# Michaelszeng/GCS-ADMM

Measured on AMD Instinct MI355X. Metric: admm_iterations_per_sec, higher is better.
Workload: dtype f64

## Files before the change

gcs_admm_amd/csrc/vertex_wg.h:

```cpp
#pragma once
#include <type_traits>

#include "gcs_math.h"
#include "step_args.h"
#include "warm_start.h"

#if defined(__HIP_DEVICE_COMPILE__)
#define WG_DEVICE 1
#else
#define WG_DEVICE 0
#endif

namespace gcs_wg {

using gcs_math::rcp;
using gcs_math::rcp1;
using gcs_math::rsqrt_nr;
using gcs_math::sqrt_nr;

#ifndef GCS_WG_THREADS
#define GCS_WG_THREADS 256
#endif
constexpr int WG_THREADS = GCS_WG_THREADS;
constexpr int WG_WAVES = WG_THREADS / 64;
// ... 160 lines not shown

struct alignas(8) WgF2 { float a, b; };

template <class T> struct WgArgs : gcsadmm_k::StepArgs<T> {
    int n_vtx;
    const int *vtx;
    const double *prox_q = nullptr, *prox_c = nullptr;
    const int *order = nullptr;
    int *unit_iters = nullptr;
};

struct Red3 { double mn, s1, s2; };

#if WG_DEVICE
template <int SH> __device__ __forceinline__ double dpp_row_shr(double x, double ident)
{
    const int ilo = __double2loint(ident), ihi = __double2hiint(ident);
    const int lo = __builtin_amdgcn_update_dpp(ilo, __double2loint(x), 0x110 + SH, 0xf, 0xf, false);
    const int hi = __builtin_amdgcn_update_dpp(ihi, __double2hiint(x), 0x110 + SH, 0xf, 0xf, false);
    return __hiloint2double(hi, lo);
}
__device__ __forceinline__ double lane_bcast(double x, int lane)
{
    return __hiloint2double(__builtin_amdgcn_readlane(__double2hiint(x), lane), __builtin_amdgcn_readlane(__double2loint(x), lane));
}
#endif

GCS_HD double wg_uniform(double x)
{
#if WG_DEVICE
    return __hiloint2double(__builtin_amdgcn_readfirstlane(__double2hiint(x)), __builtin_amdgcn_readfirstlane(__double2loint(x)));
#else
    return x;
#endif
}
GCS_HD int wg_uniform(int x)
{
#if WG_DEVICE
    return __builtin_amdgcn_readfirstlane(x);
#else
    return x;
#endif
}

template <bool VM = false> GCS_HD Red3 wg_reduce(Red3 v, double *red, int &phase)
{
#if WG_DEVICE
    v.mn = fmin(v.mn, dpp_row_shr<1>(v.mn, 1e300)); v.s1 += dpp_row_shr<1>(v.s1, 0.0); v.s2 += dpp_row_shr<1>(v.s2, 0.0);
    v.mn = fmin(v.mn, dpp_row_shr<2>(v.mn, 1e300)); v.s1 += dpp_row_shr<2>(v.s1, 0.0); v.s2 += dpp_row_shr<2>(v.s2, 0.0);
    v.mn = fmin(v.mn, dpp_row_shr<4>(v.mn, 1e300)); v.s1 += dpp_row_shr<4>(v.s1, 0.0); v.s2 += dpp_row_shr<4>(v.s2, 0.0);
    v.mn = fmin(v.mn, dpp_row_shr<8>(v.mn, 1e300)); v.s1 += dpp_row_shr<8>(v.s1, 0.0); v.s2 += dpp_row_shr<8>(v.s2, 0.0);
    Red3 w;
    w.mn = fmin(fmin(lane_bcast(v.mn, 15), lane_bcast(v.mn, 31)), fmin(lane_bcast(v.mn, 47), lane_bcast(v.mn, 63)));
    w.s1 = (lane_bcast(v.s1, 15) + lane_bcast(v.s1, 31)) + (lane_bcast(v.s1, 47) + lane_bcast(v.s1, 63));
    w.s2 = (lane_bcast(v.s2, 15) + lane_bcast(v.s2, 31)) + (lane_bcast(v.s2, 47) + lane_bcast(v.s2, 63));
    double *buf = red + phase * (3 * WG_WAVES);
    phase = phase == 2 ? 0 : phase + 1;
    const int wave = (int)threadIdx.x >> 6;
    if (((int)threadIdx.x & 63) == 0) { buf[wave * 3 + 0] = w.mn; buf[wave * 3 + 1] = w.s1; buf[wave * 3 + 2] = w.s2; }
    wg_barrier<VM>();
    Red3 r{buf[0], buf[1], buf[2]};
#pragma unroll
    for (int q = 1; q < WG_WAVES; ++q) { r.mn = fmin(r.mn, buf[3 * q]); r.s1 += buf[3 * q + 1]; r.s2 += buf[3 * q + 2]; }
    return r;
#else
    (void)red; (void)phase;
    return v;
#endif
}

GCS_HD void tri_decode(int t, int &r, int &c)
{
    r = (int)((sqrtf(8.0f * (float)t + 1.0f) - 1.0f) * 0.5f);
    if ((r + 1) * (r + 2) / 2 <= t) ++r;
    if (r * (r + 1) / 2 > t) --r;
    c = t - r * (r + 1) / 2;
}

GCS_HD int fdiv(int x, float inv) { return (int)(((float)x + 0.5f) * inv); }

GCS_HD constexpr int pki(int i, int j) { return i * (i + 1) / 2 + j; }

template <int DIM> GCS_HD void wave_ldl(double *Mq, double *rd)
{
    static_assert(DIM <= 64, "one row per lane");
#if WG_DEVICE
    const int lane = wg_tid() & 63, row = lane < DIM ? lane : DIM - 1;
    double a[DIM];
#pragma unroll
    for (int j = 0; j < DIM; ++j) a[j] = Mq[row * DIM + j];
    const double od = Mq[row * DIM + row];
    double myr = 0.0;
#pragma unroll
    for (int k = 0; k < DIM; ++k) {
        double dk = lane_bcast(a[k], k);
        const double odk = lane_bcast(od, k);
        if (!(dk > CHOL_SKIP * odk)) dk = odk > 0.0 ? CHOL_SKIP * odk : 1.0;
        const double rk = rcp(dk), col = a[k], l = col * rk;
        a[k] = l;
        if (lane == k) myr = rk;
#pragma unroll
        for (int j = k + 1; j < DIM; ++j) a[j] -= l * lane_bcast(col, j);
    }
    if (lane < DIM) {
#pragma unroll
        for (int j = 0; j < DIM - 1; ++j) Mq[lane * DIM + j] = a[j];
        rd[lane] = myr;
    }
#else
    double od[DIM], col[DIM];
    for (int k = 0; k < DIM; ++k) od[k] = Mq[k * DIM + k];
    for (int k = 0; k < DIM; ++k) {
        double dk = Mq[k * DIM + k];
        if (!(dk > CHOL_SKIP * od[k])) dk = od[k] > 0.0 ? CHOL_SKIP * od[k] : 1.0;
        const double rk = rcp(dk);
        rd[k] = rk;
        for (int i = k + 1; i < DIM; ++i) col[i] = Mq[i * DIM + k];
        for (int i = k + 1; i < DIM; ++i) {
            const double l = col[i] * rk;
            Mq[i * DIM + k] = l;
            for (int j = k + 1; j <= i; ++j) Mq[i * DIM + j] -= l * col[j];
        }
    }
#endif
}

template <int DIM> GCS_HD void wave_ldl_solve(const double *Mq, const double *rd, const double *b, double *x)
{
#if WG_DEVICE
    const int lane = wg_tid() & 63, row = lane < DIM ? lane : DIM - 1;
    double l[DIM], v = b[row];
#pragma unroll
    for (int k = 0; k < DIM - 1; ++k) l[k] = k < row ? Mq[row * DIM + k] : 0.0;
#pragma unroll
    for (int k = 0; k < DIM - 1; ++k) v -= l[k] * lane_bcast(v, k);
    v *= rd[row];
#pragma unroll
    for (int k = 1; k < DIM; ++k) l[k] = k > row ? Mq[k * DIM + row] : 0.0;
#pragma unroll
    for (int k = DIM - 1; k >= 1; --k) v -= l[k] * lane_bcast(v, k);
    if (lane < DIM) x[lane] = v;
#else
    double v[DIM];
    for (int i = 0; i < DIM; ++i) v[i] = b[i];
    for (int k = 0; k < DIM - 1; ++k)
        for (int i = k + 1; i < DIM; ++i) v[i] -= Mq[i * DIM + k] * v[k];
    for (int i = 0; i < DIM; ++i) v[i] *= rd[i];
    for (int k = DIM - 1; k >= 1; --k)
        for (int i = 0; i < k; ++i) v[i] -= Mq[k * DIM + i] * v[k];
    for (int i = 0; i < DIM; ++i) x[i] = v[i];
#endif
}

template <int DIM, bool LOWREG> GCS_HD void ldl_inverse_col(const double *Lm, const double *rd, int c, double *out, int ldo)
{
    double x[DIM];
#pragma unroll
    for (int i = 0; i < DIM; ++i) {
        double s = (i == c) ? 1.0 : 0.0;
#pragma unroll
        for (int k = 0; k < i; ++k) s -= Lm[i * DIM + k] * x[k];
        x[i] = s;
        if constexpr (DIM > 9) WG_FENCE();
    }
#pragma unroll
    for (int i = DIM - 1; i >= 0; --i) {
        double s = x[i] * rd[i];
#pragma unroll
        for (int k = i + 1; k < DIM; ++k) s -= Lm[k * DIM + i] * x[k];
        x[i] = s;
        if constexpr (LOWREG) out[i * ldo + c] = s;
        if constexpr (DIM > 9) WG_FENCE();
    }
    if constexpr (!LOWREG) {
#pragma unroll
        for (int i = 0; i < DIM; ++i) out[i * ldo + c] = x[i];
    }
}

template <int Q> GCS_HD bool soc_scaling_wb(const double *s, const double *z, double *wb, double &eta)
{
    const double ss = gcs_math::soc_det<Q>(s), zz = gcs_math::soc_det<Q>(z);
    if (!(ss > 0.0) || !(zz > 0.0)) return false;
    const double is = rsqrt_nr(ss), iz = rsqrt_nr(zz);
    double dot = 0;
    for (int k = 0; k < Q; ++k) dot += (s[k] * is) * (z[k] * iz);
    const double ig2 = 0.5 * rsqrt_nr(0.5 * (1.0 + dot));
    wb[0] = (s[0] * is + z[0] * iz) * ig2;
    for (int k = 1; k < Q; ++k) wb[k] = (s[k] * is - z[k] * iz) * ig2;
    eta = sqrt_nr((ss * is) * iz);
    return true;
}

template <int Q> GCS_HD void soc_apply_W(const double *wb, double eta, const double *x, double *y)
{
    double dd = 0;
#pragma unroll
    for (int k = 1; k < Q; ++k) dd += wb[k] * x[k];
    const double f = x[0] + dd * rcp(1.0 + wb[0]);
    y[0] = eta * (wb[0] * x[0] + dd);
#pragma unroll
    for (int k = 1; k < Q; ++k) y[k] = eta * (x[k] + wb[k] * f);
}
template <int Q> GCS_HD void soc_apply_Wi(const double *wb, double eta, const double *x, double *y)
{
    double dd = 0;
#pragma unroll
    for (int k = 1; k < Q; ++k) dd += wb[k] * x[k];
    const double ieta = rcp(eta), f = -x[0] + dd * rcp(1.0 + wb[0]);
    y[0] = ieta * (wb[0] * x[0] - dd);
#pragma unroll
    for (int k = 1; k < Q; ++k) y[k] = ieta * (x[k] + wb[k] * f);
}
template <int Q> GCS_HD void soc_apply_W2(const double *wb, double eta, const double *x, double *y)
{
    double vx = wb[0] * x[0];
#pragma unroll
    for (int k = 1; k < Q; ++k) vx -= wb[k] * x[k];
    const double ieta = rcp(eta), ie2 = ieta * ieta;
    y[0] = ie2 * (2.0 * wb[0] * vx - x[0]);
#pragma unroll
    for (int k = 1; k < Q; ++k) y[k] = ie2 * (x[k] - 2.0 * wb[k] * vx);
}

#define WG_ROWS_BEGIN_(pl, DS)                                                                                                 \
    WG_FOR_AT(rt_, (BOX ? U * 2 * N : U * m2), (pl).at(BOX ? U * 2 * N : U * m2)) {                                            \
        int u, i, jk_;                                                                                                         \
        if constexpr (BOX) { u = rt_ / (2 * N); const int ik_ = rt_ - u * (2 * N); i = ik_ / N; jk_ = ik_ - i * N; }           \
        else { u = fdiv(rt_, inv_m2); const int rem_ = rt_ - u * m2; i = rem_ >= m; jk_ = rem_ - i * m; }                      \
        double *un = UN(u);                                                                                                    \
        double ap_ = 0, ax_ = 0, adp_ = 0, adx_ = 0;                                                                           \
        if constexpr (BOX) {                                                                                                   \
            ap_ = un[W::P + i * N + jk_]; ax_ = sm[W::XV + i * N + jk_];                                                       \
            if (DS) { adp_ = un[W::DW + i * N + jk_]; adx_ = sm[W::DX + i * N + jk_]; }                                        \
        } else {                                                                                                               \
            _Pragma("unroll") for (int k_ = 0; k_ < N; ++k_) {                                                                 \
                const double a_ = A[jk_ * N + k_];                                                                             \
                ap_ += a_ * un[W::P + i * N + k_]; ax_ += a_ * sm[W::XV + i * N + k_];                                         \
                if (DS) { adp_ += a_ * un[W::DW + i * N + k_]; adx_ += a_ * sm[W::DX + i * N + k_]; }                          \
            }                                                                                                                  \
        }                                                                                                                      \
        const double yy_ = un[W::P + 2 * N], dy_ = DS ? un[W::DW + 2 * N] : 0.0;                                               \
        _Pragma("unroll") for (int rq_ = 0; rq_ < (BOX ? 4 : 2); ++rq_) {                                                      \
            const int ty = BOX ? rq_ >> 1 : rq_, j = BOX ? jk_ + (rq_ & 1) * N : jk_, ro = ty * m2 + i * m + j;                \
            const double sg_ = (BOX && (rq_ & 1)) ? -1.0 : 1.0, b_ = BC[j];                                                    \
            const double s = ty == 0 ? b_ * yy_ - sg_ * ap_ : b_ * (1.0 - yy_) - sg_ * (ax_ - ap_);                            \
            const double ds = ty == 0 ? b_ * dy_ - sg_ * adp_ : -(b_ * dy_) - sg_ * (adx_ - adp_);                             \
            (void)ds;
#define WG_ROWS_BEGIN(pl) WG_ROWS_BEGIN_(pl, false)
#define WG_ROWS_BEGIN_DS(pl) WG_ROWS_BEGIN_(pl, true)
#define WG_ROWS_END() }}

template <int N, class T, bool BOX = false, bool SPLIT = false>
GCS_HD void wg_solve_vertex(const WgArgs<T> &a, int v, double rho, double mu_scale, double *sm, int &status_out, int &iters_out,
                            double *units = nullptr)
{
    using D = WD<N>;
    using SO = WSoc<N>;
    using W = std::conditional_t<BOX, WLBox<N>, WL<N>>;
    constexpr int NW = D::NW, NX = D::NX, NB1 = D::NB1, Q = D::Q, NS = D::NS, TA = D::TA;
#ifndef GCS_WG_CONE_PAIR_MAXN
#define GCS_WG_CONE_PAIR_MAXN 3
#endif
    constexpr bool CONE_PAIR = N <= GCS_WG_CONE_PAIR_MAXN;
    const bool prox = a.prox_q != nullptr;
    const int lo = a.inc_ptr[v], d = prox ? 0 : a.inc_ptr[v + 1] - lo, d_in = prox ? 0 : a.deg_in[v], d_out = d - d_in;
    const bool sides = d > 0;
    const int p0 = a.poly_ptr[v], m = a.poly_ptr[v + 1] - p0;
    const int U = d + 1, R = 4 * m, m2 = 2 * m;
    const int US = W::unit_stride(m);
    const float inv_m2 = 1.0f / (float)m2;
    double *const UB = SPLIT ? units : sm + W::FIXED;
    auto UN = [&](int u) -> double * { return UB + u * US; };
    constexpr bool WG_VM = SPLIT;
    const int oLAM = W::ROWS, oR1 = W::ROWS + R, oR2 = W::ROWS + 2 * R;
    double *const PA = sm + W::FIXED + (SPLIT ? 0 : pad2(U * US));
    const double *A = PA, *BC = PA + pad2(m * N), *CEN = sm + W::CEN;
    double *SOC = sm + W::SOC, *SC = sm + W::SC;
    int red_phase = 0;
    WG_STAMP_INIT();
    const int deg = (4 * m + 2) * (d + 1) + 1;
    const double inv_deg = 1.0 / (double)deg;
    auto side_of = [&](int u) { return (u - 1) >= d_in ? 1 : 0; };
    auto side_lo = [&](int s) { return s ? d_in + 1 : 1; };
    auto side_hi = [&](int s) { return s ? d : d_in; };

    using WR = gcs_ws::WRec<N>;
    double *const wrec = (a.warm != nullptr && !prox) ? a.warm + a.warm_ptr[v] : nullptr;
    const int WUS = WR::unit_stride(m);
    double dtm = 0.0;
    Place pl0;
    WG_FOR_AT(t, d * NW, pl0.at(d * NW)) {
        const int e = t / NW, w = t - e * NW, edge = a.inc_edge[lo + e];
        const bool out = e >= d_in;
        const int inc = gcsadmm_k::state_column(a, lo, e, edge, out);
        double *un = UN(e + 1);
        const double Tw = gcsadmm_k::consensus_target(a, w, edge, inc, mu_scale);
        int slot = -1;
        if (w == 2 * N) slot = 2 * N;
        else if (out) slot = w;
        else if (w < N) { un[W::TF + w] = Tw; un[W::TG + N + w] = 0.0; }
        else slot = w - N;
        if (slot >= 0) {
            un[W::TG + slot] = Tw;
            if (wrec) dtm = fmax(dtm, fabs(Tw - wrec[WR::UNITS + (e + 1) * WUS + WR::TG + slot]));
        }
    }
    WG_FOR_AT(t, m * N, pl0.at(m * N)) PA[t] = a.poly_A[(size_t)p0 * N + t];
    WG_FOR_AT(j, m + N, pl0.at(m + N)) {
        if (j < m) PA[pad2(m * N) + j] = a.poly_bc[p0 + j];
        else sm[W::CEN + (j - m)] = a.center[(size_t)v * N + (j - m)];
    }
    if (prox) {
        WG_FOR(k, NX + NW) {
            sm[W::PQ + k] = a.prox_q[(size_t)v * (NX + NW) + k];
            sm[W::PC + k] = a.prox_c[(size_t)v * (NX + NW) + k];
        }
    }
    bool use_warm = false;
    double mu_ref = gcs_ws::WS_COLD_REF, ws_dT = -1.0;
    if (wrec) {
        const Red3 rt = wg_reduce<WG_VM>(Red3{-dtm, 0.0, 0.0}, sm + W::RED, red_phase);
        const bool comparable = wg_uniform((int)(wrec[0] == 1.0 && wrec[1] == rho)) != 0;
        ws_dT = wg_uniform(comparable ? -rt.mn * rho : -1.0);
        use_warm = wg_uniform((int)(comparable && ws_dT <= gcs_ws::ws_theta(wrec))) != 0;
        if (use_warm) mu_ref = wg_uniform(fmax(gcs_ws::WS_MU_MIN, gcs_ws::WS_KAPPA * ws_dT));
    }
    const bool ws_started_warm = use_warm;
    const float inv_R2 = 1.0f / (float)(R / 2);

    WG_STAMP(0);
    auto gval = [&](const double *un, int u, int k, bool wk) {
        double g = un[W::G0 + k];
        if (wk) {
            g += un[W::GU + k];
            if (u == 0 && k < 2 * N) g += k < N ? -SOC[SO::KS + 1 + k] : SOC[SO::KS + 1 + (k - N)];
        }
        return g;
    };
    auto te_tasks = [&](Place &pl, bool wk) {
        WG_FOR_AT(t, d * NW, pl.at(d * NW)) {
            const int u = 1 + t / NW, i = t - (u - 1) * NW;
            double *un = UN(u);
            double s = 0;
            if constexpr (BOX) {
                double wg = 0;
#pragma unroll
                for (int k = 0; k < NW; ++k) wg += un[W::BW + k] * gval(un, u, k, wk);
                s = -(un[W::BRS] * un[W::BW + i]) * wg;
                if (i < 2 * N) s -= un[W::BD + i] * gval(un, u, i, wk);
            } else {
#pragma unroll
                for (int k = 0; k < NW; ++k) s -= un[W::B + i * NW + k] * gval(un, u, k, wk);
            }
            un[W::TE + i] = s;
        }
    };
    auto bg_tasks = [&](Place &pl) {
        WG_FOR_AT(t, 2 * NW, pl.at(2 * NW)) {
            const int s = t / NW, i = t - s * NW;
            double acc = 0;
#pragma unroll 4
            for (int u = side_lo(s); u <= side_hi(s); ++u) acc += UN(u)[W::TE + i];
            sm[W::BG + t] = acc;
        }
        WG_FOR_AT(t, 2 * NX, pl.at(2 * NX)) {
            const int part = t / NX, c = t - part * NX, h = c / N;
            const int ulo = part ? 1 + d / 2 : 1, uhi = part ? d : d / 2;
            double acc = 0;
#pragma unroll 2
            for (int u = ulo; u <= uhi; ++u) {
                const double *un = UN(u);
                if constexpr (BOX) acc += un[W::XD + c] * un[W::TE + c] + un[W::XY + c] * un[W::TE + 2 * N];
                else {
#pragma unroll
                    for (int k = 0; k < N; ++k) acc += un[W::X + (h * N + k) * NX + c] * un[W::TE + h * N + k];
                    acc += un[W::X + 2 * N * NX + c] * un[W::TE + 2 * N];
                }
            }
            sm[W::XBG + t] = acc;
        }
    };
    auto v_tasks = [&](Place &pl) {
        WG_FOR_AT(t, 2 * NW, pl.at(2 * NW)) {
            const int s = t / NW, i = t - s * NW;
            const double *Bsi = sm + W::BSI + s * NW * NW;
            double acc = 0;
#pragma unroll
            for (int k = 0; k < NW; ++k) acc += Bsi[i * NW + k] * (sm[W::RP + s * NW + k] - sm[W::BG + s * NW + k]);
            sm[W::VV + t] = acc;
        }
    };
    auto rhs_tasks = [&](Place &pl, bool wk) {
        const double *u0 = UN(0);
        auto base_z = [&](int i) { return -gval(u0, 0, i, wk) - sm[W::VV + i] - sm[W::VV + NW + i]; };
        WG_FOR_AT(q, NX, pl.at(NX)) {
            double r = -REG_DELTA * sm[W::XV + q] - sm[W::XBG + q] - sm[W::XBG + NX + q];
            if (prox) r -= sm[W::PQ + q] * (sm[W::XV + q] + CEN[q < N ? q : q - N] - sm[W::PC + q]);
            if (wk) r -= sm[W::SOL + q];
            for (int s = 0; s < 2; ++s) {
                const double *BXs = sm + W::BXS + s * NW * NX;
#pragma unroll
                for (int i = 0; i < NW; ++i) r -= BXs[i * NX + q] * sm[W::VV + s * NW + i];
            }
            sm[W::RHS + q] = r;
        }
        WG_FOR_AT(k, N, pl.at(N))
            sm[W::RHS + NX + k] = base_z(k) + SOC[SO::CV + k] * SC[SC_GT] * rcp(SC[SC_C0]);
        WG_FOR_AT(k, N, pl.at(N))
            sm[W::RHS + NX + N + k] = base_z(k) + base_z(N + k);
        WG_FOR_AT(k, 1, pl.at(1)) sm[W::RHS + NX + 2 * N + k] = base_z(2 * N);
    };
    auto solve_head = [&](bool wk) {
        {
            Place pl;
            te_tasks(pl, wk);
            if (wk) {
                WG_FOR_AT(q, NX, pl.at(NX)) {
                    double acc = 0;
#pragma unroll 4
                    for (int u = 0; u <= d; ++u) acc += UN(u)[W::GX + q];
                    sm[W::SOL + q] = acc;
                }
            }
        }
        WG_ARRIVE(30);
        WG_SYNC();
        WG_STAMP(30);
        { Place pl; bg_tasks(pl); }
        WG_ARRIVE(31);
        WG_SYNC();
        WG_STAMP(31);
        { Place pl; v_tasks(pl); }
        WG_ARRIVE(32);
        WG_SYNC();
        WG_STAMP(32);
        { Place pl; rhs_tasks(pl, wk); }
        WG_ARRIVE(33);
        WG_SYNC();
        WG_STAMP(33);
    };
    auto cone_dir = [&](int dt_slot, bool wk, double (&xs)[Q], double (&dl)[Q]) {
        const double *u0 = UN(0);
        double wb[Q], ys[Q];
        xs[0] = SC[dt_slot];
#pragma unroll
        for (int k = 0; k < N; ++k) xs[1 + k] = u0[W::DW + k] - u0[W::DW + N + k];
#pragma unroll
        for (int k = 0; k < Q; ++k) wb[k] = SOC[SO::WB + k];
        soc_apply_W2<Q>(wb, SC[SC_ETA], xs, ys);
#pragma unroll
        for (int k = 0; k < Q; ++k) dl[k] = (wk ? SOC[SO::KS + k] : 0.0) - SOC[SO::LS + k] - ys[k];
    };
    auto solve_tail = [&](int dt_slot, bool wk) {
        WG_WAVE0() wave_ldl_solve<NB1>(sm + W::M, sm + W::PIVM, sm + W::RHS, sm + W::SOL);
        WG_ARRIVE(34);
        WG_SYNC();
        WG_STAMP(34);
        auto dzeta = [&](int i) { return i < N ? sm[W::SOL + NX + i] + sm[W::SOL + NX + N + i] : sm[W::SOL + NX + i]; };
        Place plw;
        WG_FOR_AT(t, 2 * NW, plw.at(2 * NW)) {
            const int s = t / NW, i = t - s * NW;
            const double *BXs = sm + W::BXS + s * NW * NX;
            double acc = dzeta(i) + (sm[W::RP + t] - sm[W::BG + t]);
#pragma unroll
            for (int c = 0; c < NX; ++c) acc += BXs[i * NX + c] * sm[W::SOL + c];
            sm[W::WW + t] = acc;
        }
        WG_FOR_AT(t, NX + NW + 1, plw.at(NX + NW + 1)) {
            if (t < NX) sm[W::DX + t] = sm[W::SOL + t];
            else if (t < NX + NW) UN(0)[W::DW + (t - NX)] = dzeta(t - NX);
            else {
                double acc = -SC[SC_GT];
#pragma unroll
                for (int k = 0; k < N; ++k) acc -= SOC[SO::CV + k] * sm[W::SOL + NX + k];
                SC[dt_slot] = acc * rcp(SC[SC_C0]);
            }
        }
        WG_ARRIVE(36);
        WG_SYNC();
        WG_STAMP(36);
        auto cone_bounds = [&](int l) {
            const int oDS = wk ? SO::DSS : SO::DSSA, oDL = wk ? SO::DLS : SO::DLSA;
            double xs[Q], dl[Q], bs[Q], dr[Q];
            cone_dir(dt_slot, wk, xs, dl);
            double c1c = 0, c2c = 0;
#pragma unroll
            for (int k = 0; k < Q; ++k) {
                const double sk = SOC[SO::SS + k], lk = SOC[SO::LS + k];
                SOC[oDS + k] = xs[k]; SOC[oDL + k] = dl[k];
                c1c += sk * dl[k] + lk * xs[k];
                c2c += xs[k] * dl[k];
                bs[k] = l == 1 ? lk : sk; dr[k] = l == 1 ? dl[k] : xs[k];
            }
            SC[SC_C1C] = c1c; SC[SC_C2C] = c2c;
            SC[l == 1 ? SC_AMAXC2 : SC_AMAXC] = gcs_math::soc_max_step<Q>(bs, dr);
            if (l == 2) SC[SC_AMAXC2] = gcs_math::soc_max_step<Q>(SOC + SO::LS, dl);
        };
        if constexpr (CONE_PAIR) { WG_CONE2(l) cone_bounds(l); }
        else { WG_CONE() cone_bounds(2); }
        WG_REPL_FOR(t, 2 * NW) {
            const int s = t / NW, i = t - s * NW;
            const double *Bsi = sm + W::BSI + s * NW * NW;
            double acc = 0;
#pragma unroll
            for (int k = 0; k < NW; ++k) acc += Bsi[i * NW + k] * sm[W::WW + s * NW + k];
            sm[W::DNU + t] = acc;
        }
        WG_WAVE_SYNC();
        WG_ITEM_FOR(q, i, d, NW) {
            const int u = 1 + q;
            double *un = UN(u);
            double acc = -gval(un, u, i, wk) + sm[W::DNU + side_of(u) * NW + i];
            if constexpr (BOX) {
                if (i < 2 * N) acc -= un[W::XD + i] * sm[W::DX + i];
                else {
#pragma unroll
                    for (int c = 0; c < NX; ++c) acc -= un[W::XY + c] * sm[W::DX + c];
                }
            } else if (i < 2 * N) {
                const int h = i / N;
#pragma unroll
                for (int k = 0; k < N; ++k) acc -= un[W::X + i * NX + h * N + k] * sm[W::DX + h * N + k];
            } else {
#pragma unroll
                for (int c = 0; c < NX; ++c) acc -= un[W::X + i * NX + c] * sm[W::DX + c];
            }
            un[W::RV + i] = acc;
        }
        WG_WAVE_SYNC();
        WG_ITEM_FOR(q, i, d, NW) {
            double *un = UN(1 + q);
            double acc = 0;
            if constexpr (BOX) {
                double wr = 0;
#pragma unroll
                for (int k = 0; k < NW; ++k) wr += un[W::BW + k] * un[W::RV + k];
                acc = (un[W::BRS] * un[W::BW + i]) * wr;
                if (i < 2 * N) acc += un[W::BD + i] * un[W::RV + i];
            } else {
#pragma unroll
                for (int k = 0; k < NW; ++k) acc += un[W::B + i * NW + k] * un[W::RV + k];
            }
            un[W::DW + i] = acc;
        }
        WG_ARRIVE(39);
        WG_SYNC();
        WG_STAMP(39);
    };

    int status = -1, it = 0, it_total = 0, stalled = 0;
    bool saved = false, init_pending = true;
#define WG_FAIL_OR_RESTART()                                                                                                   \
    {                                                                                                                          \
        if (!use_warm) break;                                                                                                  \
        it_total += it; it = -1;                                                                                               \
        use_warm = false; mu_ref = gcs_ws::WS_COLD_REF; init_pending = true;                                                   \
        WG_SYNC();                                                                                                             \
        continue;                                                                                                              \
    }
    for (it = 0;; ++it) {
    if (init_pending) {
        init_pending = false; stalled = 0; saved = false;
        Place pls;
        if (use_warm) {
            const double *wu = wrec + WR::UNITS;
            WG_FOR_AT(t, U * NW, pls.at(U * NW)) {
                const int u = t / NW, k = t - u * NW;
                UN(u)[W::P + k] = wu[u * WUS + WR::P + k];
            }
            WG_FOR_AT(t, U * (R / 2), pls.at(U * (R / 2))) {
                const int u = fdiv(t, inv_R2), r2 = t - u * (R / 2);
                const WgF2 v = reinterpret_cast<const WgF2 *>(wu + u * WUS + WR::LAM)[r2];
                UN(u)[oLAM + 2 * r2] = (double)v.a; UN(u)[oLAM + 2 * r2 + 1] = (double)v.b;
            }
            WG_FOR_AT(t, 2 * U, pls.at(2 * U)) UN(t >> 1)[W::LB + (t & 1)] = wu[(t >> 1) * WUS + WR::LB + (t & 1)];
            WG_FOR_AT(k, NX + 2 * NW, pls.at(NX + 2 * NW)) {
                if (k < NX) sm[W::XV + k] = wrec[WR::XV + k];
                else sm[W::NU + (k - NX)] = wrec[WR::NU + (k - NX)];
            }
        } else {
            WG_FOR_AT(t, U * NW, pls.at(U * NW)) {
                const int u = t / NW, k = t - u * NW;
                double val = 0.0;
                if (k == 2 * N) val = u == 0 ? 0.5 : 0.5 / (double)(side_of(u) ? d_out : d_in);
                UN(u)[W::P + k] = val;
            }
            WG_FOR_AT(k, NX + 2 * NW, pls.at(NX + 2 * NW)) {
                if (k < NX) sm[W::XV + k] = 0.0;
                else sm[W::NU + (k - NX)] = 0.0;
            }
            WG_ONE() {
                SC[SC_T] = 1.0;
                SOC[SO::LS] = 1.0;
                for (int k = 1; k < Q; ++k) SOC[SO::LS + k] = 0.0;
            }
        }
        WG_SYNC();
    }
        const bool first_warm = use_warm && it == 0;
        double acc = 0.0; int bad = 0;
        Place plr;
        WG_ROWS_BEGIN(plr)
            const double is = rcp1(s);
            if (it == 0 && !use_warm) un[oLAM + ro] = is;
            const double l = un[oLAM + ro];
            un[oR1 + ro] = l * is;
            acc += s * l;
            if (!(s > 0.0)) bad = 1;
        WG_ROWS_END()
        WG_FOR_AT(u, U, plr.at(U)) {
            double *un = UN(u);
            const double yy = un[W::P + 2 * N], s5 = yy, s6 = 1.0 - yy;
            if (it == 0 && !use_warm) { un[W::LB] = rcp1(s5); un[W::LB + 1] = rcp1(s6); }
            acc += s5 * un[W::LB] + s6 * un[W::LB + 1];
            if (!(s5 > 0.0) || !(s6 > 0.0)) bad = 1;
        }
        WG_FOR_AT(tg, U * NW, plr.at(U * NW)) {
            const int u = tg / NW, k = tg - u * NW;
            double *un = UN(u);
            const double *p = un + W::P;
            double g;
            if (u == 0) {
                g = sm[W::NU + k] + sm[W::NU + NW + k] + REG_DELTA * p[k];
                if (prox) {
                    const double *qz = sm + W::PQ + NX, *cz = sm + W::PC + NX;
                    const double yy = p[2 * N];
                    if (k < 2 * N) g += qz[k] * (p[k] + yy * CEN[k < N ? k : k - N] - cz[k]);
                    else {
                        g += qz[2 * N] * (yy - cz[2 * N]);
#pragma unroll
                        for (int c = 0; c < 2 * N; ++c) g += CEN[c < N ? c : c - N] * qz[c] * (p[c] + yy * CEN[c < N ? c : c - N] - cz[c]);
                    }
                }
            }
            else {
                const bool out = side_of(u);
                const double *tg_ = un + W::TG, *nu = sm + W::NU + (out ? NW : 0);
                const double yy = p[2 * N];
                if (k < N) g = rho * (p[k] + yy * CEN[k] - tg_[k]);
                else if (k < 2 * N) g = out ? rho * (p[k] + yy * CEN[k - N] - tg_[k]) : 0.0;
                else {
                    g = rho * (yy - tg_[2 * N]) + a.eps_edge;
#pragma unroll
                    for (int c = 0; c < N; ++c) {
                        g += CEN[c] * rho * (p[c] + yy * CEN[c] - tg_[c]);
                        if (out) g += CEN[c] * rho * (p[N + c] + yy * CEN[c] - tg_[N + c]);
                    }
                }
                g += REG_DELTA * p[k] - nu[k];
            }
            un[W::G0 + k] = g;
        }
        WG_CONE() {
            const double *u0 = UN(0);
            if (first_warm) {
                double uu = 0;
                for (int k = 0; k < N; ++k) { const double uk = u0[W::P + k] - u0[W::P + N + k]; uu += uk * uk; }
                const double tn = 0.5 * (mu_ref + sqrt_nr(mu_ref * mu_ref + 4.0 * uu)), itn = rcp(tn);
                SC[SC_T] = tn;
                SOC[SO::LS] = 1.0;
                for (int k = 0; k < N; ++k) SOC[SO::LS + 1 + k] = -(u0[W::P + k] - u0[W::P + N + k]) * itn;
            }
            SOC[SO::SS] = SC[SC_T];
            for (int k = 0; k < N; ++k) SOC[SO::SS + 1 + k] = u0[W::P + k] - u0[W::P + N + k];
            for (int k = 0; k < Q; ++k) acc += SOC[SO::SS + k] * SOC[SO::LS + k];
            if (!gcs_math::soc_interior<Q>(SOC + SO::SS)) bad = 1;
        }
        WG_ARRIVE(1);
        const Red3 r0 = wg_reduce<WG_VM>(Red3{bad ? -1.0 : 1.0, acc, 0.0}, sm + W::RED, red_phase);
        WG_STAMP(1);
        const double gap = wg_uniform(r0.s1);
        const double mu = wg_uniform(r0.mn < 0.0 ? 0.0 / 0.0 : gap * inv_deg);
        WG_FENCE();
        if (wrec != nullptr && !saved && it >= 1 && mu <= gcs_ws::WS_SAVE * mu_ref) {
            saved = true;
            double *wu = wrec + WR::UNITS;
            Place plv;
            WG_FOR_AT(t, U * NW, plv.at(U * NW)) {
                const int u = t / NW, k = t - u * NW;
                wu[u * WUS + WR::P + k] = UN(u)[W::P + k];
                if (u > 0) wu[u * WUS + WR::TG + k] = UN(u)[W::TG + k];
            }
            WG_FOR_AT(t, U * (R / 2), plv.at(U * (R / 2))) {
                const int u = fdiv(t, inv_R2), r2 = t - u * (R / 2);
                WgF2 v; v.a = (float)UN(u)[oLAM + 2 * r2]; v.b = (float)UN(u)[oLAM + 2 * r2 + 1];
                reinterpret_cast<WgF2 *>(wu + u * WUS + WR::LAM)[r2] = v;
            }
            WG_FOR_AT(t, 2 * U, plv.at(2 * U)) wu[(t >> 1) * WUS + WR::LB + (t & 1)] = UN(t >> 1)[W::LB + (t & 1)];
            WG_FOR_AT(k, NX + 2 * NW, plv.at(NX + 2 * NW)) {
                if (k < NX) wrec[WR::XV + k] = sm[W::XV + k];
                else wrec[WR::NU + (k - NX)] = sm[W::NU + (k - NX)];
            }
            WG_ONE() { wrec[0] = 1.0; wrec[1] = rho; }
        }
        WG_FENCE();
        {
            const bool conv = !first_warm && (mu <= a.ipm_tol || (stalled && mu <= 1e3 * a.ipm_tol));
            bool stop = conv;
            status = conv ? ((use_warm && !(mu <= a.ipm_tol)) ? -7 : 0) : -1;
            if (!(mu > 0.0)) { stop = true; status = -3; }
// ... 280 lines not shown
#pragma unroll 4
                for (int u = side_lo(s); u <= side_hi(s); ++u) {
                    const double *un = UN(u);
                    acc2 += (un[W::BRS] * un[W::BW + i]) * un[W::BQ + c];
                    if (i == c) acc2 += un[W::BD + c] * un[W::XD + c];
                }
            } else {
#pragma unroll 4
                for (int u = side_lo(s); u <= side_hi(s); ++u) acc2 += UN(u)[W::K + q];
            }
            sm[W::BXS + tt] = acc2;
        }
        WG_FOR_AT(tp0, 2 * NXT, plq.at(2 * NXT)) {
            const int part = tp0 / NXT;
            int r, c;
            tri_decode(tp0 - part * NXT, r, c);
            const int tp = part * NX * NX + r * NX + c, h = r / N;
            (void)h;
            const int ulo = part ? 1 + d / 2 : 1, uhi = part ? d : d / 2;
            double acc2 = 0;
#pragma unroll 2
            for (int u = ulo; u <= uhi; ++u) {
                const double *un = UN(u);
                if constexpr (BOX) {
                    acc2 += (un[W::BRS] * un[W::BQ + r]) * un[W::BQ + c];
                    if (r == c) acc2 += (un[W::XD + r] * un[W::XD + r]) * un[W::BD + r];
                } else {
#pragma unroll
                    for (int k = 0; k < N; ++k) acc2 += un[W::X + (h * N + k) * NX + r] * un[W::K + (h * N + k) * NX + c];
                    acc2 += un[W::X + 2 * N * NX + r] * un[W::K + 2 * N * NX + c];
                }
            }
            sm[W::XBX + tp] = acc2;
        }
        WG_FOR_AT(tt, NX * N, plq.at(NX * N)) {
            const int r = tt / N, c = (r / N) * N + (tt - r * N);
            double acc2 = 0;
            if constexpr (BOX) {
                if (c == r) {
#pragma unroll 4
                    for (int u = 0; u <= d; ++u) acc2 += UN(u)[W::XD + r];
                }
            } else {
#pragma unroll 4
                for (int u = 0; u <= d; ++u) acc2 += UN(u)[W::X + r * NX + c];
            }
            sm[W::XS + tt] = acc2;
        }
        WG_FOR_AT(tt, 2 * NW, plq.at(2 * NW)) {
            const int s = tt / NW, k = tt - s * NW;
            double acc2 = UN(0)[W::P + k];
#pragma unroll 4
            for (int u = side_lo(s); u <= side_hi(s); ++u) acc2 -= UN(u)[W::P + k];
            sm[W::RP + tt] = acc2;
        }
        if (!first_warm) bg_tasks(plq);
        WG_ARRIVE(6);
        WG_SYNC();
        WG_STAMP(6);
        Place ply;
        if (sides) {
            WG_FIRST_WAVES(sd, 2) wave_ldl<NW>(sm + W::BS + sd * NW * NW, sm + W::PIVS + sd * NW);
            WG_ARRIVE(7);
            WG_SYNC();
            WG_STAMP(7);
            WG_FOR(t, 2 * NW) {
                const int s = t / NW, c = t - s * NW;
                ldl_inverse_col<NW, (!BOX && NW > 9)>(sm + W::BS + s * NW * NW, sm + W::PIVS + s * NW, c, sm + W::BSI + s * NW * NW, NW);
            }
            WG_SYNC();
            WG_FOR_AT(t, 2 * NW * NX, ply.at(2 * NW * NX)) {
                const int s = t / (NW * NX), ic = t - s * NW * NX, i = ic / NX, c = ic - i * NX;
                const double *Bsi = sm + W::BSI + s * NW * NW, *BXs = sm + W::BXS + s * NW * NX;
                double acc2 = 0;
#pragma unroll
                for (int k = 0; k < NW; ++k) acc2 += Bsi[i * NW + k] * BXs[k * NX + c];
                sm[W::BS + s * NW * NW + ic] = acc2;
            }
        } else {
            WG_FOR(t, 2 * NW * NW) { sm[W::BSI + t] = 0.0; sm[W::BS + t] = 0.0; }
            WG_SYNC();
        }
        if (!first_warm) v_tasks(ply);
        WG_ARRIVE(9);
        WG_SYNC();
        WG_STAMP(9);
        {
            const double *YS0 = sm + W::BS, *YS1 = sm + W::BS + NW * NW, *u0 = UN(0);
            auto x0 = [&](int i, int c) {
                if constexpr (BOX) return i == c ? u0[W::XD + c] : (i == 2 * N ? u0[W::XY + c] : 0.0);
                else return u0[W::X + i * NX + c];
            };
            auto k0 = [&](int hi, int lo) {
                if constexpr (BOX) return hi == lo ? (hi < 2 * N ? u0[W::KD + hi] : u0[W::KYY]) : (hi == 2 * N ? u0[W::KY + lo] : 0.0);
                else return u0[W::K + hi * NW + lo];
            };
            auto zx = [&](int i, int c) { return x0(i, c) + YS0[i * NX + c] + YS1[i * NX + c]; };
            auto zz = [&](int i, int k) {
                const int hi = i > k ? i : k, lo = i > k ? k : i;
                return k0(hi, lo) + sm[W::BSI + hi * NW + lo] + sm[W::BSI + NW * NW + hi * NW + lo];
            };
            Place plm;
            WG_FOR_AT(t, NX * (NX + 1) / 2, plm.at(NX * (NX + 1) / 2)) {
                int r, c;
                tri_decode(t, r, c);
                double val = (r == c ? REG_DELTA + (prox ? sm[W::PQ + r] : 0.0) : 0.0) - sm[W::XBX + r * NX + c] - sm[W::XBX + NX * NX + r * NX + c];
                if (r / N == c / N) val -= sm[W::XS + r * N + (c - (c / N) * N)];
#pragma unroll
                for (int k = 0; k < NW; ++k)
                    val += sm[W::BXS + k * NX + r] * YS0[k * NX + c] + sm[W::BXS + NW * NX + k * NX + r] * YS1[k * NX + c];
                sm[W::M + r * NB1 + c] = val;
            }
            WG_FOR_AT(t, NW * NX, plm.at(NW * NX)) {
                const int i = t / NX, c = t - i * NX;
                double val = zx(i, c);
                if (i >= N && i < 2 * N) val += zx(i - N, c);
                sm[W::M + (NX + i) * NB1 + c] = val;
            }
            WG_FOR_AT(t, NW * (NW + 1) / 2, plm.at(NW * (NW + 1) / 2)) {
                int i, k;
                tri_decode(t, i, k);
                const bool rz2 = i >= N && i < 2 * N, cz2 = k >= N && k < 2 * N;
                double val = zz(i, k);
                if (cz2) val += zz(i, k - N);
                if (rz2) val += zz(i - N, k);
                if (rz2 && cz2) val += zz(i - N, k - N);
                if (i < N && k < N) val += SOC[SO::SU + i * N + k];
                sm[W::M + (NX + i) * NB1 + NX + k] = val;
            }
            if (!first_warm) rhs_tasks(plm, false);
        }
        WG_ARRIVE(10);
        WG_SYNC();
        WG_STAMP(10);
        WG_WAVE0() wave_ldl<NB1>(sm + W::M, sm + W::PIVM);
        WG_ARRIVE(11);
        WG_SYNC();
        WG_STAMP(11);
        WG_STAMP(12);
        double rmax = 0.0, c1 = 0.0, c2 = 0.0, amax_cone = 1e300;
        double sigmu;
        if (first_warm) {
            Place plb;
            WG_ROWS_BEGIN(plb)
                un[oR1 + ro] = 0.0;
                un[oR2 + ro] = rcp1(s);
            WG_ROWS_END()
            WG_FOR_AT(u, U, plb.at(U)) { double *un = UN(u); un[W::KB] = 0.0; un[W::KB + 1] = 0.0; }
            sigmu = mu_ref;
            WG_ARRIVE(14);
            WG_SYNC();
            WG_STAMP(14);
        } else {
        solve_tail(SC_DTA, false);
        WG_STAMP(13);
        Place plb;
        WG_ROWS_BEGIN_DS(plb)
            const double l = un[oLAM + ro], is = rcp1(s);
            const double q = ds * is, dl = -l - l * q;
            rmax = fmax(rmax, fmax(-q, 1.0 + q));
            c1 += s * dl + l * ds; c2 += ds * dl;
            un[oR1 + ro] = ds * dl;
            un[oR2 + ro] = is;
        WG_ROWS_END()
        WG_FOR_AT(u, U, plb.at(U)) {
            double *un = UN(u);
            const double yy = un[W::P + 2 * N], dy = un[W::DW + 2 * N];
            const double s5 = yy, s6 = 1.0 - yy, l5 = un[W::LB], l6 = un[W::LB + 1];
            const double q5 = dy * rcp1(s5), q6 = -dy * rcp1(s6);
            const double dl5 = -l5 - l5 * q5, dl6 = -l6 - l6 * q6;
            rmax = fmax(rmax, fmax(fmax(-q5, 1.0 + q5), fmax(-q6, 1.0 + q6)));
            c1 += s5 * dl5 + l5 * dy + s6 * dl6 - l6 * dy; c2 += dy * dl5 - dy * dl6;
            un[W::KB] = dy * dl5; un[W::KB + 1] = -dy * dl6;
        }
        WG_CONE() { amax_cone = fmin(SC[SC_AMAXC], SC[SC_AMAXC2]); c1 += SC[SC_C1C]; c2 += SC[SC_C2C]; }
        WG_ARRIVE(14);
        const Red3 rb = wg_reduce<WG_VM>(Red3{fmin(rmax > 0.0 ? rcp1(rmax) : 1e300, amax_cone), c1, c2}, sm + W::RED, red_phase);
        WG_STAMP(14);
        {
            const double al = fmin(1.0, rb.mn);
            const double mu_aff = (gap + al * rb.s1 + al * al * rb.s2) * inv_deg;
            double sig = mu_aff * rcp(mu);
            sig = sig < 0 ? 0 : (sig > 1 ? 1 : sig);
            sig = sig * sig * sig;
            sigmu = wg_uniform(sig * mu);
        }
        }
        WG_CONE() {
            double wb[Q], a1[Q], a2[Q], pr[Q], qv[Q], xs[Q], lt[Q], ss[Q];
            const double eta = SC[SC_ETA];
#pragma unroll
            for (int k = 0; k < Q; ++k) { wb[k] = SOC[SO::WB + k]; xs[k] = SOC[SO::DSSA + k]; lt[k] = SOC[SO::LT + k]; ss[k] = SOC[SO::SS + k]; }
            soc_apply_Wi<Q>(wb, eta, xs, a1);
#pragma unroll
            for (int k = 0; k < Q; ++k) xs[k] = SOC[SO::DLSA + k];
            soc_apply_W<Q>(wb, eta, xs, a2);
            double dsum = 0;
#pragma unroll
            for (int k = 0; k < Q; ++k) dsum += a1[k] * a2[k];
            pr[0] = dsum;
#pragma unroll
            for (int k = 1; k < Q; ++k) pr[k] = a1[0] * a2[k] + a2[0] * a1[k];
            const double det = gcs_math::soc_det<Q>(lt);
            double ld1 = 0;
#pragma unroll
            for (int k = 1; k < Q; ++k) ld1 += lt[k] * pr[k];
            qv[0] = (lt[0] * pr[0] - ld1) * rcp(det);
            const double ilt0 = rcp(lt[0]);
#pragma unroll
            for (int k = 1; k < Q; ++k) qv[k] = (pr[k] - qv[0] * lt[k]) * ilt0;
            const double smd = sigmu * rcp(gcs_math::soc_det<Q>(ss));
            soc_apply_Wi<Q>(wb, eta, qv, a1);
#pragma unroll
            for (int i = 0; i < Q; ++i) SOC[SO::KS + i] = smd * (i == 0 ? ss[0] : -ss[i]) - (first_warm ? 0.0 : a1[i]);
            SC[SC_GT] = 1.0 - SOC[SO::KS];
        }
        Place plg;
        WG_FOR_AT(t, U * 2 * N, plg.at(U * 2 * N)) {
            const int u = t / (2 * N), q = t - u * (2 * N), i = q / N, k = q - i * N;
            double *un = UN(u);
            const double *ea = un + oR1, *eb = ea + m2, *ia = un + oR2, *ib = ia + m2;
            double su = 0, sx = 0;
            if constexpr (BOX) {
                const int jp = i * m + k, jn = jp + N;
                const double kbp = (sigmu - eb[jp]) * ib[jp], kbn = (sigmu - eb[jn]) * ib[jn];
                su = ((sigmu - ea[jp]) * ia[jp] - kbp) - ((sigmu - ea[jn]) * ia[jn] - kbn);
                sx = kbp - kbn;
            } else {
#pragma unroll 4
                for (int j = 0; j < m; ++j) {
                    const double kb = (sigmu - eb[i * m + j]) * ib[i * m + j], aj = A[j * N + k];
                    su += aj * ((sigmu - ea[i * m + j]) * ia[i * m + j] - kb);
                    sx += aj * kb;
                }
            }
            un[W::GU + q] = su;
            un[W::GX + q] = sx;
        }
        WG_FOR_AT(u, U, plg.at(U)) {
            double *un = UN(u);
            const double *ea = un + oR1, *eb = ea + m2, *ia = un + oR2, *ib = ia + m2;
            double s = 0;
#pragma unroll 4
            for (int j = 0; j < m2; ++j) s += BC[j >= m ? j - m : j] * ((sigmu - eb[j]) * ib[j] - (sigmu - ea[j]) * ia[j]);
            const double yy = un[W::P + 2 * N];
            un[W::GU + 2 * N] = s - (sigmu - un[W::KB]) * rcp1(yy) + (sigmu - un[W::KB + 1]) * rcp1(1.0 - yy);
        }
        WG_ARRIVE(16);
        WG_SYNC();
        WG_STAMP(16);
        solve_head(true);
        solve_tail(SC_DT, true);
        WG_STAMP(18);
        rmax = 0.0;
        Place pld;
        WG_ROWS_BEGIN_DS(pld)
            const double l = un[oLAM + ro];
            const double ip = rcp1(s * l), is = l * ip, il = s * ip;
            const double dl = (sigmu - un[oR1 + ro]) * un[oR2 + ro] - l - (l * is) * ds;
            un[oR2 + ro] = dl;
            rmax = fmax(rmax, fmax(-ds * is, -dl * il));
        WG_ROWS_END()
        WG_FOR_AT(u, U, pld.at(U)) {
            double *un = UN(u);
            const double yy = un[W::P + 2 * N], dy = un[W::DW + 2 * N];
            const double s5 = yy, s6 = 1.0 - yy, l5 = un[W::LB], l6 = un[W::LB + 1];
            const double i5 = rcp1(s5), i6 = rcp1(s6);
            const double dl5 = (sigmu - un[W::KB]) * i5 - l5 - l5 * i5 * dy, dl6 = (sigmu - un[W::KB + 1]) * i6 - l6 + l6 * i6 * dy;
            un[W::DLB] = dl5; un[W::DLB + 1] = dl6;
            rmax = fmax(rmax, fmax(fmax(-dy * i5, -dl5 * rcp1(l5)), fmax(dy * i6, -dl6 * rcp1(l6))));
        }
        amax_cone = 1e300;
        WG_CONE() amax_cone = fmin(SC[SC_AMAXC], SC[SC_AMAXC2]);
        WG_ARRIVE(19);
        const Red3 rd = wg_reduce<WG_VM>(Red3{fmin(rmax > 0.0 ? rcp1(rmax) : 1e300, amax_cone), 0.0, 0.0}, sm + W::RED, red_phase);
        WG_STAMP(19);
        WG_CONE() {
            double al = fmin(1.0, 0.99 * rd.mn);
            for (int tries = 0; tries < 40; ++tries) {
                double s2[Q], l2[Q];
#pragma unroll
                for (int k = 0; k < Q; ++k) { s2[k] = SOC[SO::SS + k] + al * SOC[SO::DSS + k]; l2[k] = SOC[SO::LS + k] + al * SOC[SO::DLS + k]; }
                if (gcs_math::soc_interior<Q>(s2) && gcs_math::soc_interior<Q>(l2)) break;
                al *= 0.7;
            }
            SC[SC_ALPHA] = al;
        }
        WG_ARRIVE(20);
        WG_SYNC();
        WG_STAMP(20);
        const double alpha = wg_uniform(SC[SC_ALPHA]);
        stalled = alpha < 1e-3;
        Place plu;
        WG_ROWS_BEGIN(plu)
            (void)s;
            un[oLAM + ro] += alpha * un[oR2 + ro];
        WG_ROWS_END()
        WG_FOR_AT(t, U * NW, plu.at(U * NW)) {
            const int u = t / NW, k = t - u * NW;
            double *un = UN(u);
            un[W::P + k] += alpha * un[W::DW + k];
        }
        WG_FOR_AT(t, 2 * U, plu.at(2 * U)) {
            double *un = UN(t >> 1);
            un[W::LB + (t & 1)] += alpha * un[W::DLB + (t & 1)];
        }
        WG_FOR_AT(t, NX + 2 * NW, plu.at(NX + 2 * NW)) {
            if (t < NX) sm[W::XV + t] += alpha * sm[W::DX + t];
            else sm[W::NU + (t - NX)] += alpha * sm[W::DNU + (t - NX)];
        }
        WG_CONE() {
            SC[SC_T] += alpha * SC[SC_DT];
            for (int k = 0; k < Q; ++k) SOC[SO::LS + k] += alpha * SOC[SO::DLS + k];
        }
        WG_ARRIVE(21);
        WG_SYNC();
        WG_STAMP(21);
    }
#undef WG_FAIL_OR_RESTART
    it_total += it;
    if (wrec != nullptr) {
        WG_ONE() {
            if (status != 0) wrec[0] = 0.0;
            else gcs_ws::ws_learn(wrec, use_warm, ws_started_warm && !use_warm, ws_dT, it);
        }
    }
    status_out = status;
    iters_out = it_total;
    WG_STAMP(22);
    WG_SYNC();
    if (status != 0) return;
    Place plo;
    WG_FOR_AT(t, d * NW, plo.at(d * NW)) {
        const int e = t / NW, w = t - e * NW;
        const bool out = e >= d_in;
        const int inc = gcsadmm_k::state_column(a, lo, e, a.inc_edge + lo, out);
        const double *un = UN(e + 1), *p = un + W::P;
        const double yy = p[2 * N];
        double val;
        if (w == 2 * N) val = yy;
        else if (w < N) val = out ? p[w] + yy * CEN[w] : un[W::TF + w];
        else val = out ? p[w] + yy * CEN[w - N] : p[w - N] + yy * CEN[w - N];
        a.copy[(size_t)w * a.NI + inc] = (T)val;
    }
    WG_FOR_AT(k, NX, plo.at(NX)) {
        const int c = k < N ? k : k - N;
        const double *u0 = UN(0);
        a.xv[(size_t)v * NX + k] = sm[W::XV + k] + CEN[c];
        a.zv[(size_t)v * NX + k] = u0[W::P + k] + u0[W::P + 2 * N] * CEN[c];
    }
    WG_ONE() a.yv[v] = UN(0)[W::P + 2 * N];
}

}
```

Measured before the change: 9974.

## Run reduced KKT solve in a single wavefront with register shuffles

Adds a wave-level solve path that does the affine and corrector Newton step's head, LDL solve and tail entirely inside wave 0. Vectors live in per-lane registers and are exchanged with ds_bpermute and lane broadcasts, replacing several workgroup barriers and shared-memory round-trips. The cone step-bounds computation is hoisted into a reusable lambda and run after the wave solve. The path is gated to 512-thread workgroups, non-box, non-split, N≤3 and d*NW≤64. It risks idling the other waves and adds register pressure.

New measurement: 9732, median of 2. 2.4% lower.

```diff
diff --git a/gcs_admm_amd/csrc/vertex_wg.h b/gcs_admm_amd/csrc/vertex_wg.h
--- a/gcs_admm_amd/csrc/vertex_wg.h
+++ b/gcs_admm_amd/csrc/vertex_wg.h
@@ -336,6 +336,40 @@
 #endif
 }
 
+struct WaveV {
+#if WG_DEVICE
+    double v;
+    GCS_HD double &operator[](int) { return v; }
+    GCS_HD double operator[](int) const { return v; }
+#else
+    double v[64];
+    double &operator[](int l) { return v[l]; }
+    double operator[](int l) const { return v[l]; }
+#endif
+};
+GCS_HD double wave_shfl(const WaveV &x, int src)
+{
+#if WG_DEVICE
+    const int ad = src << 2;
+    return __hiloint2double(__builtin_amdgcn_ds_bpermute(ad, __double2hiint(x.v)), __builtin_amdgcn_ds_bpermute(ad, __double2loint(x.v)));
+#else
+    return x.v[src];
+#endif
+}
+GCS_HD double wave_bcast(const WaveV &x, int k)
+{
+#if WG_DEVICE
+    return lane_bcast(x.v, k);
+#else
+    return x.v[k];
+#endif
+}
+#if WG_DEVICE
+#define WAVE_LANES(l) if (const int l = gcs_wg::wg_tid() & 63; true)
+#else
+#define WAVE_LANES(l) for (int l = 0; l < 64; ++l)
+#endif
+
 template <int DIM, bool LOWREG> GCS_HD void ldl_inverse_col(const double *Lm, const double *rd, int c, double *out, int ldo)
 {
     double x[DIM];
@@ -450,6 +484,12 @@
     const bool prox = a.prox_q != nullptr;
     const int lo = a.inc_ptr[v], d = prox ? 0 : a.inc_ptr[v + 1] - lo, d_in = prox ? 0 : a.deg_in[v], d_out = d - d_in;
     const bool sides = d > 0;
+#ifndef GCS_WG_WAVE_SOLVE
+#define GCS_WG_WAVE_SOLVE 3
+#endif
+    constexpr bool WAVE_OK = WG_THREADS == 512 && !BOX && !SPLIT && N <= 3;
+    const bool wave_fit = WAVE_OK && wg_uniform((int)(!prox && d > 0 && d * NW <= 64)) != 0;
+    const bool wave_aff = (GCS_WG_WAVE_SOLVE & 1) != 0 && wave_fit, wave_cor = (GCS_WG_WAVE_SOLVE & 2) != 0 && wave_fit;
     const int p0 = a.poly_ptr[v], m = a.poly_ptr[v + 1] - p0;
     const int U = d + 1, R = 4 * m, m2 = 2 * m;
     const int US = W::unit_stride(m);
@@ -636,6 +676,27 @@
 #pragma unroll
         for (int k = 0; k < Q; ++k) dl[k] = (wk ? SOC[SO::KS + k] : 0.0) - SOC[SO::LS + k] - ys[k];
     };
+    auto cone_bounds = [&](int l, int dt_slot, bool wk) {
+        const int oDS = wk ? SO::DSS : SO::DSSA, oDL = wk ? SO::DLS : SO::DLSA;
+        double xs[Q], dl[Q], bs[Q], dr[Q];
+        cone_dir(dt_slot, wk, xs, dl);
+        double c1c = 0, c2c = 0;
+#pragma unroll
+        for (int k = 0; k < Q; ++k) {
+            const double sk = SOC[SO::SS + k], lk = SOC[SO::LS + k];
+            SOC[oDS + k] = xs[k]; SOC[oDL + k] = dl[k];
+            c1c += sk * dl[k] + lk * xs[k];
+            c2c += xs[k] * dl[k];
+            bs[k] = l == 1 ? lk : sk; dr[k] = l == 1 ? dl[k] : xs[k];
+        }
+        SC[SC_C1C] = c1c; SC[SC_C2C] = c2c;
+        SC[l == 1 ? SC_AMAXC2 : SC_AMAXC] = gcs_math::soc_max_step<Q>(bs, dr);
+        if (l == 2) SC[SC_AMAXC2] = gcs_math::soc_max_step<Q>(SOC + SO::LS, dl);
+    };
+    auto cone_step_bounds = [&](int dt_slot, bool wk) {
+        if constexpr (CONE_PAIR) { WG_CONE2(l) cone_bounds(l, dt_slot, wk); }
+        else { WG_CONE() cone_bounds(2, dt_slot, wk); }
+    };
     auto solve_tail = [&](int dt_slot, bool wk) {
         WG_WAVE0() wave_ldl_solve<NB1>(sm + W::M, sm + W::PIVM, sm + W::RHS, sm + W::SOL);
         WG_ARRIVE(34);
@@ -664,25 +725,7 @@
         WG_ARRIVE(36);
         WG_SYNC();
         WG_STAMP(36);
-        auto cone_bounds = [&](int l) {
-            const int oDS = wk ? SO::DSS : SO::DSSA, oDL = wk ? SO::DLS : SO::DLSA;
-            double xs[Q], dl[Q], bs[Q], dr[Q];
-            cone_dir(dt_slot, wk, xs, dl);
-            double c1c = 0, c2c = 0;
-#pragma unroll
-            for (int k = 0; k < Q; ++k) {
-                const double sk = SOC[SO::SS + k], lk = SOC[SO::LS + k];
-                SOC[oDS + k] = xs[k]; SOC[oDL + k] = dl[k];
-                c1c += sk * dl[k] + lk * xs[k];
-                c2c += xs[k] * dl[k];
-                bs[k] = l == 1 ? lk : sk; dr[k] = l == 1 ? dl[k] : xs[k];
-            }
-            SC[SC_C1C] = c1c; SC[SC_C2C] = c2c;
-            SC[l == 1 ? SC_AMAXC2 : SC_AMAXC] = gcs_math::soc_max_step<Q>(bs, dr);
-            if (l == 2) SC[SC_AMAXC2] = gcs_math::soc_max_step<Q>(SOC + SO::LS, dl);
-        };
-        if constexpr (CONE_PAIR) { WG_CONE2(l) cone_bounds(l); }
-        else { WG_CONE() cone_bounds(2); }
+        cone_step_bounds(dt_slot, wk);
         WG_REPL_FOR(t, 2 * NW) {
             const int s = t / NW, i = t - s * NW;
             const double *Bsi = sm + W::BSI + s * NW * NW;
@@ -731,6 +774,170 @@
         WG_ARRIVE(39);
         WG_SYNC();
         WG_STAMP(39);
+    };
+    auto wave_solve = [&](bool head, int dt_slot, bool wk) {
+        if constexpr (WAVE_OK) {
+        const int nin = d_in, nout = d - d_in, jsd = nin > nout ? nin : nout, dh = d / 2, jxb = d - dh;
+        auto qa = [&](int l) { const int q = l / NW; return q < d ? q : d - 1; };
+        auto sa = [&](int l) { return l < NW ? 0 : 1; };
+        auto ia = [&](int l) { return l - (l / NW) * NW; };
+        WaveV Br[NW], Sr[NW], Xr[NX], Lf[NB1 - 1], Lb[NB1 - 1], rdv, bg, xbg, gxs, te, vv, rv;
+        WAVE_LANES(l) {
+            const int q = qa(l), i = ia(l), s = sa(l), row = l < NB1 ? l : NB1 - 1;
+            const double *un = UN(1 + q), *Bsi = sm + W::BSI + s * NW * NW;
+#pragma unroll
+            for (int k = 0; k < NW; ++k) { Br[k][l] = un[W::B + i * NW + k]; Sr[k][l] = Bsi[i * NW + k]; }
+#pragma unroll
+            for (int c = 0; c < NX; ++c) Xr[c][l] = un[W::X + i * NX + c];
+#pragma unroll
+            for (int k = 0; k < NB1 - 1; ++k) {
+                Lf[k][l] = k < row ? sm[W::M + row * NB1 + k] : 0.0;
+                Lb[k][l] = k + 1 > row ? sm[W::M + (k + 1) * NB1 + row] : 0.0;
+            }
+            rdv[l] = sm[W::PIVM + row];
+            if (head) {
+                double s_ = 0;
+#pragma unroll
+                for (int k = 0; k < NW; ++k) s_ -= Br[k][l] * gval(un, 1 + q, k, wk);
+                te[l] = s_;
+                if (wk) {
+                    const int qx = l < NX ? l : NX - 1;
+                    double acc = 0;
+#pragma unroll 4
+                    for (int u = 0; u <= d; ++u) acc += UN(u)[W::GX + qx];
+                    gxs[l] = acc;
+                }
+            } else {
+                bg[l] = sm[W::BG + (l < 2 * NW ? l : 2 * NW - 1)];
+                rv[l] = sm[W::RHS + row];
+            }
+        }
+        if (head) {
+            WAVE_LANES(l) {
+                const int s = sa(l), i = ia(l), cnt = s ? nout : nin, lo_ = side_lo(s);
+                double acc = 0;
+                for (int j = 0; j < jsd; ++j) {
+                    const int u = lo_ + (j < cnt ? j : 0);
+                    const double x = wave_shfl(te, ((u <= d ? u : d) - 1) * NW + i);
+                    if (j < cnt) acc += x;
+                }
+                bg[l] = acc;
+                const int part = l < NX ? 0 : 1, c = l - (l / NX) * NX, h = c / N, ulo = part ? 1 + dh : 1, cntp = part ? d - dh : dh;
+                double ax = 0;
+                for (int j = 0; j < jxb; ++j) {
+                    const int u0_ = ulo + (j < cntp ? j : 0), u = u0_ <= d ? u0_ : d;
+                    const double *un = UN(u);
+                    double tv[N + 1];
+#pragma unroll
+                    for (int k = 0; k < N; ++k) tv[k] = wave_shfl(te, (u - 1) * NW + h * N + k);
+                    tv[N] = wave_shfl(te, (u - 1) * NW + 2 * N);
+                    if (j < cntp) {
+#pragma unroll
+                        for (int k = 0; k < N; ++k) ax += un[W::X + (h * N + k) * NX + c] * tv[k];
+                        ax += un[W::X + 2 * N * NX + c] * tv[N];
+                    }
+                }
+                xbg[l] = ax;
+            }
+            WAVE_LANES(l) {
+                const int s = sa(l);
+                double acc = 0;
+#pragma unroll
+                for (int k = 0; k < NW; ++k) {
+                    const double b0 = wave_bcast(bg, k), b1 = wave_bcast(bg, NW + k);
+                    acc += Sr[k][l] * (sm[W::RP + s * NW + k] - (s ? b1 : b0));
+                }
+                vv[l] = acc;
+            }
+            double vb[2 * NW];
+#pragma unroll
+            for (int t = 0; t < 2 * NW; ++t) vb[t] = wave_bcast(vv, t);
+            WAVE_LANES(l) {
+                const int j = l < NB1 ? l : NB1 - 1, qx = j < NX ? j : 0;
+                const int z0 = j < NX ? 0 : (j < NX + N ? j - NX : (j < NX + 2 * N ? j - NX - N : 2 * N)), z1 = j < NX + N ? 0 : (j < NX + 2 * N ? j - NX : 0);
+                const double xa = wave_shfl(xbg, qx), xb = wave_shfl(xbg, NX + qx);
+                const double va0 = wave_shfl(vv, z0), vb0 = wave_shfl(vv, NW + z0), va1 = wave_shfl(vv, z1), vb1 = wave_shfl(vv, NW + z1);
+                const double *u0 = UN(0);
+                double r;
+                if (j < NX) {
+                    r = -REG_DELTA * sm[W::XV + j] - xa - xb;
+                    if (wk) r -= gxs[l];
+                    for (int s = 0; s < 2; ++s) {
+                        const double *BXs = sm + W::BXS + s * NW * NX;
+#pragma unroll
+                        for (int i = 0; i < NW; ++i) r -= BXs[i * NX + j] * vb[s * NW + i];
+                    }
+                } else if (j < NX + N) r = (-gval(u0, 0, z0, wk) - va0 - vb0) + SOC[SO::CV + z0] * SC[SC_GT] * rcp(SC[SC_C0]);
+                else if (j < NX + 2 * N) r = (-gval(u0, 0, z0, wk) - va0 - vb0) + (-gval(u0, 0, z1, wk) - va1 - vb1);
+                else r = -gval(u0, 0, 2 * N, wk) - va0 - vb0;
+                rv[l] = r;
+            }
+        }
+#pragma unroll
+        for (int k = 0; k < NB1 - 1; ++k) {
+            const double b = wave_bcast(rv, k);
+            WAVE_LANES(l) rv[l] -= Lf[k][l] * b;
+        }
+        WAVE_LANES(l) rv[l] *= rdv[l];
+#pragma unroll
+        for (int k = NB1 - 1; k >= 1; --k) {
+            const double b = wave_bcast(rv, k);
+            WAVE_LANES(l) rv[l] -= Lb[k - 1][l] * b;
+        }
+        double sx[NB1];
+#pragma unroll
+        for (int c = 0; c < NB1; ++c) sx[c] = wave_bcast(rv, c);
+        WaveV ww, dnu, re;
+        WAVE_LANES(l) {
+            const int s = sa(l), i = ia(l);
+            const double za = wave_shfl(rv, NX + i), zb = wave_shfl(rv, NX + N + (i < N ? i : 0));
+            const double dz = i < N ? za + zb : za;
+            const double *BXs = sm + W::BXS + s * NW * NX;
+            double acc = dz + (sm[W::RP + s * NW + i] - bg[l]);
+#pragma unroll
+            for (int c = 0; c < NX; ++c) acc += BXs[i * NX + c] * sx[c];
+            ww[l] = acc;
+            if (l < NX) sm[W::DX + l] = rv[l];
+            if (l < NW) UN(0)[W::DW + l] = dz;
+            if (l == 0) {
+                double a_ = -SC[SC_GT];
+#pragma unroll
+                for (int k = 0; k < N; ++k) a_ -= SOC[SO::CV + k] * sx[NX + k];
+                SC[dt_slot] = a_ * rcp(SC[SC_C0]);
+            }
+        }
+        WAVE_LANES(l) {
+            const int s = sa(l);
+            double acc = 0;
+#pragma unroll
+            for (int k = 0; k < NW; ++k) {
+                const double w0 = wave_bcast(ww, k), w1 = wave_bcast(ww, NW + k);
+                acc += Sr[k][l] * (s ? w1 : w0);
+            }
+            dnu[l] = acc;
+            if (l < 2 * NW) sm[W::DNU + l] = acc;
+        }
+        WAVE_LANES(l) {
+            const int q = qa(l), i = ia(l), u = 1 + q;
+            double acc = -gval(UN(u), u, i, wk) + wave_shfl(dnu, side_of(u) * NW + i);
+            if (i < 2 * N) {
+                const int h = i / N;
+#pragma unroll
+                for (int k = 0; k < N; ++k) acc -= (h ? Xr[N + k][l] : Xr[k][l]) * (h ? sx[N + k] : sx[k]);
+            } else {
+#pragma unroll
+                for (int c = 0; c < NX; ++c) acc -= Xr[c][l] * sx[c];
+            }
+            re[l] = acc;
+        }
+        WAVE_LANES(l) {
+            const int q = qa(l), i = ia(l);
+            double acc = 0;
+#pragma unroll
+            for (int k = 0; k < NW; ++k) acc += Br[k][l] * wave_shfl(re, q * NW + k);
+            if (l < d * NW) UN(1 + q)[W::DW + i] = acc;
+        }
+        } else { (void)head; (void)dt_slot; (void)wk; }
     };
 
     int status = -1, it = 0, it_total = 0, stalled = 0;
@@ -1317,9 +1524,18 @@
             WG_SYNC();
             WG_STAMP(14);
         } else {
-        solve_tail(SC_DTA, false);
+        if (wave_aff) {
+            WG_WAVE0() wave_solve(false, SC_DTA, false);
+            WG_ARRIVE(40);
+            WG_SYNC();
+            WG_STAMP(40);
+        } else solve_tail(SC_DTA, false);
         WG_STAMP(13);
         Place plb;
+        if (wave_aff) {
+            cone_step_bounds(SC_DTA, false);
+            WG_WAVE_SYNC();
+        }
         WG_ROWS_BEGIN_DS(plb)
             const double l = un[oLAM + ro], is = rcp1(s);
             const double q = ds * is, dl = -l - l * q;
@@ -1414,11 +1630,22 @@
         WG_ARRIVE(16);
         WG_SYNC();
         WG_STAMP(16);
-        solve_head(true);
-        solve_tail(SC_DT, true);
+        if (wave_cor) {
+            WG_WAVE0() wave_solve(true, SC_DT, true);
+            WG_ARRIVE(41);
+            WG_SYNC();
+            WG_STAMP(41);
+        } else {
+            solve_head(true);
+            solve_tail(SC_DT, true);
+        }
         WG_STAMP(18);
         rmax = 0.0;
         Place pld;
+        if (wave_cor) {
+            cone_step_bounds(SC_DT, true);
+            WG_WAVE_SYNC();
+        }
         WG_ROWS_BEGIN_DS(pld)
             const double l = un[oLAM + ro];
             const double ip = rcp1(s * l), is = l * ip, il = s * ip;
```
